# taaha-khan/2023-CompaCT-Image-Compression

Hardware: AMD Instinct MI355X
Metric: MPixels/s encode+decode, 12-bit 512x512 CT batch, bytes-exact (higher is better)
Workload: dtype u16

## Files before the change

### 2023-compact-image-compression_amd/csrc/deflate_kernels.hip

```cpp
#include <hip/hip_runtime.h>
#include <cstring>
#include <algorithm>

#include "cct_internal.h"
#include "wave_device.h"
#include "../../include/compact_hip.h"

namespace cct {
namespace {

constexpr int MIN_MATCH = 3, MAX_MATCH = 258, WSIZE = 32768;
constexpr int MIN_LOOKAHEAD = MAX_MATCH + MIN_MATCH + 1;
constexpr int MAX_DIST = WSIZE - MIN_LOOKAHEAD;
constexpr int TOO_FAR = 4096;
constexpr int BLOCK_SYMS = 16383;
constexpr int BLOCK_SYMS_ML9 = 32767;
constexpr int L_CODES = 286, D_CODES = 30, BL_CODES = 19, HEAP_SIZE = 2 * L_CODES + 1;
constexpr int END_BLOCK = 256, MAX_BITS = 15, MAX_BL_BITS = 7;
constexpr uint32_t Z_FILTERED = 1, Z_HUFFMAN_ONLY = 2, Z_RLE = 3, Z_FIXED = 4;
__host__ __device__ __forceinline__ bool short_pass(uint32_t strategy) { return strategy == Z_HUFFMAN_ONLY || strategy == Z_RLE; }

__constant__ uint8_t c_extra_lbits[29] = {0,0,0,0,0,0,0,0,1,1,1,1,2,2,2,2,3,3,3,3,4,4,4,4,5,5,5,5,0};
__constant__ uint8_t c_extra_dbits[30] = {0,0,0,0,1,1,2,2,3,3,4,4,5,5,6,6,7,7,8,8,9,9,10,10,11,11,12,12,13,13};
__constant__ uint8_t c_extra_blbits[19] = {0,0,0,0,0,0,0,0,0,0,0,0,0,0,0,0,2,3,7};
// ... 831 lines not shown
		const bool prev_eq = p >= 2 ? (rw >> 15) != 0 : (p == 1 && (rw0 & 0x7FFFu) >= 2u);
		const uint32_t run = rw & 0x7FFFu;
		uint32_t rec = 0, nxt = blk_end, cnt = 0;
		if (p < L) {
			const bool m = prev_eq && run >= (uint32_t)MIN_MATCH;
			rec = m ? (run << 8) | (1u << 17) : 0u;
			nxt = p + (m ? run : 1u);
			cnt = 1;
		}
		a.rec32[base + p] = rec;
#pragma unroll
		for (int r = 0; r < 6; r++) {
			const bool inside = nxt < blk_end;
			const int j = inside ? (int)(nxt - wb * 64) : lane;
			const uint32_t n2 = __shfl(nxt, j), c2 = __shfl(cnt, j);
			if (inside) { nxt = n2; cnt += c2; }
		}
		a.exit_pos[base + p] = (nxt - blk_end) | (cnt << 16);
	}
}

template <uint32_t BS>
__global__ void __launch_bounds__(256) dfl_huff_symbols_kernel(DeflateArgs a)
{
	const int s = blockIdx.y;
	const uint32_t L = a.in_sizes[s];
	const size_t base = (size_t)s * a.in_stride;
	const uint32_t *in4 = reinterpret_cast<const uint32_t *>(a.in + base);
	uint4 *sym4 = reinterpret_cast<uint4 *>(a.sym + base);
	uint32_t *bend = a.blk_end + (size_t)s * a.max_blocks, *btop = a.blk_top + (size_t)s * a.max_blocks;
	if (blockIdx.x == 0 && threadIdx.x == 0) a.total_syms[s] = L;
	const uint32_t nq = (L + 3) / 4;
	for (uint32_t q = blockIdx.x * blockDim.x + threadIdx.x; q < nq; q += gridDim.x * blockDim.x) {
		const uint32_t w = in4[q], p0 = 4 * q;
		uint32_t v[4];
#pragma unroll
		for (int k = 0; k < 4; k++) {
			const uint32_t p = p0 + (uint32_t)k;
			v[k] = p < L ? (w >> (8 * k)) & 255u : 0u;
			if (p < L && p % BS == BS - 1) { bend[p / BS] = p + 1; btop[p / BS] = p; }
		}
		sym4[q] = make_uint4(v[0], v[1], v[2], v[3]);
	}
}

#ifndef CCT_WALK_T
#define CCT_WALK_T 256
#endif
constexpr int WALK_T = CCT_WALK_T;
__global__ void __launch_bounds__(WALK_T) dfl_walk_kernel(DeflateArgs a, int n)
{
	__shared__ uint32_t s_land[WALK_T];
	__shared__ uint32_t s_wsum[WALK_T / 64];
	const int s = blockIdx.x;
	(void)n;
	const uint32_t L = a.in_sizes[s];
	const size_t base = (size_t)s * a.in_stride;
	const size_t bbase = (size_t)s * dfl_blk_words(a.in_stride);
	const uint32_t *exit_rec = a.exit_pos + base;
	const int tid = threadIdx.x;
	const uint32_t seg = (((L + WALK_T - 1) / WALK_T) + 63) & ~63u;
	const uint32_t seg_end = min(L, (uint32_t)(tid + 1) * seg);
	uint32_t start = min(L, (uint32_t)tid * seg), land = start, cnt = 0;
	auto hop_through = [&]() {
		uint32_t cur = start, c = 0;
		while (cur < seg_end) { const uint32_t e = exit_rec[cur]; c += e >> 16; cur = (cur & ~63u) + 64u + (e & 0xFFFFu); }
		land = cur; cnt = c;
	};
	hop_through();
	for (;;) {
		__syncthreads();
		s_land[tid] = land;
		__syncthreads();
		const uint32_t pl = tid ? s_land[tid - 1] : 0u;
		const bool moved = tid > 0 && pl != start;
		if (!__syncthreads_or(moved)) break;
		if (moved) { start = pl; hop_through(); }
	}
	uint32_t total;
	uint32_t syms = wg_excl_scan<WALK_T / 64>(cnt, s_wsum, total);
	if (tid == 0) a.total_syms[s] = total;
	for (uint32_t cur = start; cur < seg_end;) {
		const uint32_t b = cur >> 6;
		a.blk_entry[bbase + b] = cur;
		a.blk_symbase[bbase + b] = syms;
		const uint32_t e = exit_rec[cur];
		syms += e >> 16;
		cur = (cur & ~63u) + 64u + (e & 0xFFFFu);
	}
}

template <uint32_t BS>
__global__ void __launch_bounds__(256) dfl_symbols_kernel(DeflateArgs a)
{
	const int s = blockIdx.y;
	const uint32_t L = a.in_sizes[s];
	const uint8_t *in = a.in + (size_t)s * a.in_stride;
	const size_t base = (size_t)s * a.in_stride;
	const size_t bbase = (size_t)s * dfl_blk_words(a.in_stride);
	const uint32_t nblk64 = (L + 63) / 64;
	const int lane = threadIdx.x & 63;
	uint32_t *sym = a.sym + base;
	uint32_t *bend = a.blk_end + (size_t)s * a.max_blocks, *btop = a.blk_top + (size_t)s * a.max_blocks;
	const uint32_t lazy = short_pass(a.strategy) ? 0u : 1u;
	const uint32_t wb_step = gridDim.x * (blockDim.x >> 6), wb_last = nblk64 ? nblk64 - 1 : 0;
	struct Req { uint32_t entry, symbase, rec; uint8_t lit0; };
	auto request = [&](uint32_t wb) {
		const uint32_t wbc = min(wb, wb_last), pc = min(wbc * 64 + lane, L - 1);
		return Req{a.blk_entry[bbase + wbc], a.blk_symbase[bbase + wbc], a.rec32[base + pc], in[pc]};
	};
	const uint32_t wb0 = blockIdx.x * (blockDim.x >> 6) + (threadIdx.x >> 6);
	Req nx = nblk64 ? request(wb0) : Req{0xFFFFFFFFu, 0, 0, 0};
	for (uint32_t wb = wb0; wb < nblk64; wb += wb_step) {
		const uint32_t p = wb * 64 + lane;
		const Req cur_req = nx;
		nx = request(wb + wb_step);
		const uint32_t entry = cur_req.entry, symbase = cur_req.symbase;
		uint32_t rec = cur_req.rec;
		const uint8_t lit0 = cur_req.lit0;
		if (entry == 0xFFFFFFFFu) continue;
		if (p >= L) rec = 0;
		const uint32_t k = rec & 0xFFu, len = (rec >> 8) & 0x1FFu, dist = rec >> 17;
		const uint32_t nxt = len ? p + k + len : p + 1;
		const uint32_t cnt = len ? k + 1 : 1;
		const uint64_t jump = __ballot(len != 0);
		const uint32_t nvalid = min(64u, L - wb * 64);
		uint64_t visited = 0;
		uint32_t cur = (uint32_t)__builtin_amdgcn_readfirstlane((int)(entry - wb * 64));
		while (cur < nvalid) {
			const uint64_t rest = jump >> cur;
			if (!rest) { visited |= ~0ull << cur; break; }
			const int d = __ffsll((long long)rest) - 1;
			visited |= (d >= 63 ? ~0ull : ((2ull << d) - 1ull)) << cur;
			cur = (uint32_t)__builtin_amdgcn_readlane((int)nxt, (int)cur + d) - wb * 64;
		}
		if (nvalid < 64) visited &= (1ull << nvalid) - 1ull;
		const bool mine = (visited >> lane) & 1ull;
		const uint32_t v = mine ? cnt : 0u;
		uint32_t off = symbase + wave_incl_scan(v) - v;
		if (mine) {
			if (p == L - 1) a.postloop_lit[s] = 1;
			for (uint32_t t = 0; t < (len ? k : 1u); t++, off++) {
				sym[off] = t ? in[p + t] : lit0;
				if (off % BS == BS - 1) { bend[off / BS] = p + t + 1; btop[off / BS] = p + t + lazy; }
			}
			if (len) {
				sym[off] = (len - MIN_MATCH) | (dist << 16);
				if (off % BS == BS - 1) { bend[off / BS] = p + k + len; btop[off / BS] = p + k + lazy; }
			}
		}
	}
}

struct TreeScratch {
	uint16_t freq[HEAP_SIZE], dad[HEAP_SIZE], len[HEAP_SIZE], code[L_CODES + 2];
	uint16_t dfreq[2 * D_CODES + 1], ddad[2 * D_CODES + 1], dlen[2 * D_CODES + 1], dcode[D_CODES + 2];
	uint16_t bfreq[2 * BL_CODES + 1], bdad[2 * BL_CODES + 1], blen[2 * BL_CODES + 1], bcode[BL_CODES + 1];
	alignas(16) uint32_t heap[HEAP_SIZE + 11];
	uint32_t bl_count[MAX_BITS + 1];
	uint16_t next_code[MAX_BITS + 1];
	int heap_len, heap_max, max_code, overflow, lmax, dmax;
	uint32_t opt_len, static_len, dyn_body_bits;
	uint32_t hdr_bits[160];
	uint32_t hdr_nbits;
	int ntok, btype, max_blindex;
	uint8_t extra_l[29], extra_d[30], extra_bl[19], bl_order[19];
	__device__ __forceinline__ uint32_t *hist_l() { return heap; }
	__device__ __forceinline__ uint32_t *hist_d() { return heap + L_CODES + 2; }
	__device__ __forceinline__ uint8_t *length_code() { return reinterpret_cast<uint8_t *>(dad); }
	__device__ __forceinline__ uint8_t *dist_code() { return reinterpret_cast<uint8_t *>(dad) + 256; }
	__device__ __forceinline__ uint16_t *tok() { return dad; }
};
static_assert(sizeof(TreeScratch) <= 8192, "13 tree waves per CU: keep the working set around 8 KB");
static_assert(HEAP_SIZE >= L_CODES + D_CODES, "token list fits dad[]");
static_assert((HEAP_SIZE + 1) * 4 >= (L_CODES + 2 + D_CODES) * 4 && HEAP_SIZE * 2 >= 768, "aliases fit");
__device__ __forceinline__ uint32_t static_llen(int n) { return n <= 143 ? 8u : n <= 255 ? 9u : n <= 279 ? 7u : 8u; }

typedef __attribute__((address_space(3))) uint16_t lds_u16;
struct TreeView { lds_u16 *freq, *dad, *len, *code; };

__device__ __forceinline__ void pqdownheap(TreeScratch &S, int k, int hl)
{
	const uint32_t v = S.heap[k];
	for (int j = k << 1; j <= hl; j = k << 1) {
		const uint2 pr = *reinterpret_cast<const uint2 *>(&S.heap[j]);
		const int right = (j < hl && pr.y <= (pr.x | 1023u)) ? 1 : 0;
		const uint32_t e = right ? pr.y : pr.x;
		if (v <= (e | 1023u)) break;
		S.heap[k] = e;
		k = j + right;
	}
	S.heap[k] = v;
}

__device__ __forceinline__ TreeView view_of(TreeScratch &S, int kind)
{
	if (kind == 0) return TreeView{(lds_u16 *)S.freq, (lds_u16 *)S.dad, (lds_u16 *)S.len, (lds_u16 *)S.code};
	if (kind == 1) return TreeView{(lds_u16 *)S.dfreq, (lds_u16 *)S.ddad, (lds_u16 *)S.dlen, (lds_u16 *)S.dcode};
	return TreeView{(lds_u16 *)S.bfreq, (lds_u16 *)S.bdad, (lds_u16 *)S.blen, (lds_u16 *)S.bcode};
}
__device__ __forceinline__ int elems_of(int kind) { return kind == 0 ? L_CODES : kind == 1 ? D_CODES : BL_CODES; }

__device__ void tree_leaves(TreeScratch &S, int kind)
{
	const TreeView t = view_of(S, kind);
	const int lane = threadIdx.x, elems = elems_of(kind);
	const uint64_t lt_mask = (1ull << lane) - 1ull;
	int max_code = -1;
	uint32_t nleaf = 0;
	for (int n0 = 0; n0 < elems; n0 += 64) {
		const int n = n0 + lane;
		const uint32_t f = n < elems ? t.freq[n] : 0u;
		const uint64_t bal = __ballot(f != 0);
		if (f != 0) S.heap[1 + nleaf + (uint32_t)__popcll(bal & lt_mask)] = (f << 15) | (uint32_t)n;
		else if (n < elems) t.len[n] = 0;
		if (bal) max_code = n0 + 63 - __clzll((long long)bal);
		nleaf += (uint32_t)__popcll(bal);
	}
	if (lane == 0) { S.heap_len = (int)nleaf; S.max_code = max_code; }
}

constexpr int TREE_SIFTS = 8;
__device__ void tree_heap(TreeScratch &S, int kind)
{
	const TreeView t = view_of(S, kind);
	const int lane = threadIdx.x;
	int max_code = S.max_code, h = S.heap_len;
	while (h < 2) {
		const int node = max_code < 2 ? ++max_code : 0;
		h++;
		if (lane == 0) {
			t.freq[node] = 1; S.opt_len--;
			S.heap[h] = (1u << 15) | (uint32_t)node;
			if (kind == 0) S.static_len -= static_llen(node);
			else if (kind == 1) S.static_len -= 5;
		}
	}
	__syncthreads();
	for (int d = 31 - __clz(h >> 1); d >= 0; d--) {
		const int lo = 1 << d, hi = min((2 << d) - 1, h >> 1);
		for (int n0 = lo; n0 <= hi; n0 += 64) {
			if (n0 + lane <= hi) pqdownheap(S, n0 + lane, h);
			__builtin_amdgcn_wave_barrier();
		}
	}
	if (lane < TREE_SIFTS) {
		uint32_t v = 0, k = 1, hl = 0, w = 0;
		bool moving = false;
		const uint32_t sink = HEAP_SIZE + 3 + lane;
		auto tick = [&]() {
			const uint32_t j = k << 1;
			const uint2 pr = *reinterpret_cast<const uint2 *>(&S.heap[j]);
			const uint32_t right = (j < hl && pr.y <= (pr.x | 1023u)) ? 1u : 0u;
			const uint32_t e = right ? pr.y : pr.x;
			const bool go = moving && j <= hl && v > (e | 1023u);
			w = go ? e : v;
			uint32_t at = moving ? k : sink;
			asm volatile("" : "+v"(at), "+v"(w));
			S.heap[at] = w;
			k = go ? j + right : k;
			moving = go;
			__builtin_amdgcn_wave_barrier();
		};
		auto start = [&](int slot, uint32_t x) {
			const bool me = lane == slot;
			v = me ? x : v; k = me ? 1u : k; hl = me ? (uint32_t)h : hl; moving = moving || me;
		};
		int node = elems_of(kind), hm = HEAP_SIZE, slot = 0;
		uint32_t en = S.heap[1];
		for (;;) {
			while (__ballot(moving && ((uint32_t)h >> (__clz(k | 1u) - __clz(h))) == k)) tick();
			h--;
			start(slot, S.heap[h + 1]);
			tick();
			const uint32_t em = (uint32_t)__builtin_amdgcn_readlane((int)w, slot);
			const uint32_t f = (en >> 15) + (em >> 15);
			const uint32_t dn = (en >> 10) & 31u, dm = (em >> 10) & 31u;
			const uint32_t d = (dn >= dm ? dn : dm) + 1;
			if (lane == 0) {
				S.heap[hm - 1] = en; S.heap[hm - 2] = em;
				t.freq[node] = (uint16_t)f;
				t.dad[en & 1023u] = t.dad[em & 1023u] = (uint16_t)node;
			}
			hm -= 2;
			slot = (slot + 1) & (TREE_SIFTS - 1);
			tick();
			start(slot, (f << 15) | (d << 10) | (uint32_t)node);
			tick();
			en = (uint32_t)__builtin_amdgcn_readlane((int)w, slot);
			slot = (slot + 1) & (TREE_SIFTS - 1);
			node++;
			if (h < 2) break;
			tick();
		}
		while (__ballot(moving)) tick();
		if (lane == 0) {
			S.heap[--hm] = en;
			S.heap_len = h; S.heap_max = hm;
			S.max_code = max_code;
		}
	}
}

__device__ void tree_depths(TreeScratch &S, int kind)
{
	const TreeView t = view_of(S, kind);
	const int lane = threadIdx.x;
	const int max_length = kind == 2 ? MAX_BL_BITS : MAX_BITS;
	const int base = kind == 0 ? 257 : 0;
	const int max_code = S.max_code, heap_max = S.heap_max;
	const uint32_t root = S.heap[heap_max];
	constexpr uint16_t UNKNOWN = 0xFFFF;
	for (int h = heap_max + 1 + lane; h < HEAP_SIZE; h += 64) t.len[S.heap[h] & 1023u] = UNKNOWN;
	if (lane == 0) t.len[root & 1023u] = 0;
	if (lane <= MAX_BITS) S.bl_count[lane] = 0;
	__syncthreads();
	for (bool again = true; again;) {
		again = false;
		for (int h0 = heap_max + 1; h0 < HEAP_SIZE; h0 += 64) {
			const int h = h0 + lane;
			bool unknown = false;
			if (h < HEAP_SIZE) {
				const int n = (int)(S.heap[h] & 1023u);
				if (t.len[n] == UNKNOWN) {
					const uint32_t ld = t.len[t.dad[n]];
					if (ld == UNKNOWN) unknown = true;
					else t.len[n] = (uint16_t)min(ld + 1u, (uint32_t)max_length);
				}
			}
			if (__ballot(unknown)) again = true;
		}
		__syncthreads();
	}
	int overflow = 0;
	for (int h0 = heap_max + 1; h0 < HEAP_SIZE; h0 += 64) {
		const int h = h0 + lane;
		const bool clamped = h < HEAP_SIZE && t.len[t.dad[S.heap[h] & 1023u]] == (uint32_t)max_length;
		overflow += (int)__popcll(__ballot(clamped));
	}
	uint32_t o = 0, st = 0;
	for (int n = lane; n <= max_code; n += 64) {
		const uint32_t f = t.freq[n];
		if (f == 0) continue;
		const uint32_t bits = t.len[n];
		atomicAdd(&S.bl_count[bits], 1u);
		uint32_t xbits = 0;
		if (n >= base) xbits = kind == 0 ? S.extra_l[n - base] : kind == 1 ? S.extra_d[n] : S.extra_bl[n];
		o += f * (bits + xbits);
		if (kind == 0) st += f * (static_llen(n) + xbits);
		else if (kind == 1) st += f * (5u + xbits);
	}
	o = wave_sum(o); st = wave_sum(st);
	if (lane == 0) { S.overflow = overflow; S.opt_len += o; S.static_len += st; }
}

__device__ void tree_fix(TreeScratch &S, int kind)
{
	const TreeView t = view_of(S, kind);
	const int max_length = kind == 2 ? MAX_BL_BITS : MAX_BITS;
	const int max_code = S.max_code;
	int overflow = S.overflow;
	if (overflow > 0) {
		int bits, n, m, h = HEAP_SIZE;
		do {
			bits = max_length - 1;
			while (S.bl_count[bits] == 0) bits--;
			S.bl_count[bits]--; S.bl_count[bits + 1] += 2; S.bl_count[max_length]--;
			overflow -= 2;
		} while (overflow > 0);
		for (bits = max_length; bits != 0; bits--) {
			n = (int)S.bl_count[bits];
			while (n != 0) {
				m = (int)(S.heap[--h] & 1023u);
				if (m > max_code) continue;
				if ((uint32_t)t.len[m] != (uint32_t)bits) {
					S.opt_len += ((uint32_t)bits - t.len[m]) * t.freq[m];
					t.len[m] = (uint16_t)bits;
				}
				n--;
			}
		}
	}
	uint32_t code = 0;
	for (int bits = 1; bits <= MAX_BITS; bits++) { code = (code + S.bl_count[bits - 1]) << 1; S.next_code[bits] = (uint16_t)code; }
}

__device__ void tree_codes(TreeScratch &S, int kind)
{
	const TreeView t = view_of(S, kind);
	const int lane = threadIdx.x, max_code = S.max_code;
	const uint64_t lt_mask = (1ull << lane) - 1ull;
	uint32_t seen[MAX_BITS + 1];
#pragma unroll
	for (int b = 1; b <= MAX_BITS; b++) seen[b] = S.next_code[b];
	for (int n0 = 0; n0 <= max_code; n0 += 64) {
		const int n = n0 + lane;
		const int len = n <= max_code ? (int)t.len[n] : 0;
		uint32_t mine = 0;
#pragma unroll
		for (int b = 1; b <= MAX_BITS; b++) {
			const uint64_t bal = __ballot(len == b);
			if (len == b) mine = seen[b] + (uint32_t)__popcll(bal & lt_mask);
			seen[b] += (uint32_t)__popcll(bal);
		}
		if (len != 0) t.code[n] = (uint16_t)(__brev(mine) >> (32 - len));
	}
}

__device__ void scan_tree_wave(TreeScratch &S, const TreeView &t, int max_code)
{
	const int lane = threadIdx.x;
	constexpr int NCH = (L_CODES + 63) / 64;
	const int n_el = max_code + 1;
	uint32_t v[NCH];
	uint64_t startmask[NCH];
#pragma unroll
	for (int c = 0; c < NCH; c++) {
		const int n = c * 64 + lane;
		v[c] = n < n_el ? (uint32_t)t.len[n] : 0xFFFFu;
		const uint32_t before = n == 0 ? 0xFFFFFFFFu : (uint32_t)t.len[max(n - 1, 0)];
		startmask[c] = __ballot(n < n_el && v[c] != before);
	}
	uint16_t *tk = S.tok();
	uint32_t base = (uint32_t)S.ntok;
#pragma unroll
	for (int c = 0; c < NCH; c++) {
		if (c * 64 >= n_el) break;
		const int n = c * 64 + lane;
		const bool start = (startmask[c] >> lane) & 1ull;
		uint32_t R = 0;
		if (start) {
			int nxt = n_el;
			const uint64_t rest = lane < 63 ? startmask[c] >> (lane + 1) : 0ull;
			if (rest) nxt = n + (int)__ffsll((long long)rest);
			else {
#pragma unroll
				for (int c2 = NCH - 1; c2 > c; c2--) if (startmask[c2]) nxt = min(nxt, c2 * 64 + (int)__ffsll((long long)startmask[c2]) - 1);
			}
			R = (uint32_t)(nxt - n);
		}
		const uint32_t val = v[c];
		uint32_t nlit_head = 0, nrep6 = 0, tail_lit = 0, tail_sym = 0xFFFFFFFFu, nbig = 0;
		if (start) {
			if (val != 0) {
				if (R < 4) nlit_head = R;
				else if (R <= 6) { nlit_head = 1; tail_sym = 16u | ((R - 4u) << 5); }
				else {
					nlit_head = 1; nrep6 = 1 + (R - 7u) / 6u;
					const uint32_t r = (R - 7u) % 6u;
					if (r < 3) tail_lit = r; else tail_sym = 16u | ((r - 3u) << 5);
				}
			} else {
				nbig = R / 138u;
				const uint32_t r = R % 138u;
				if (r < 3) tail_lit = r;
				else if (r <= 10) tail_sym = 17u | ((r - 3u) << 5);
				else tail_sym = 18u | ((r - 11u) << 5);
			}
		}
		const uint32_t ntok = nlit_head + nrep6 + nbig + tail_lit + (tail_sym != 0xFFFFFFFFu ? 1u : 0u);
		uint32_t chunk_tok;
		const uint32_t ex = wave_excl_scan(ntok, chunk_tok);
		if (start) {
			uint32_t w = base + ex;
			for (uint32_t i = 0; i < nlit_head; i++) tk[w++] = (uint16_t)val;
			for (uint32_t i = 0; i < nrep6; i++) tk[w++] = (uint16_t)(16u | (3u << 5));
			for (uint32_t i = 0; i < nbig; i++) tk[w++] = (uint16_t)(18u | (127u << 5));
			for (uint32_t i = 0; i < tail_lit; i++) tk[w++] = (uint16_t)val;
			if (tail_sym != 0xFFFFFFFFu) tk[w++] = (uint16_t)tail_sym;
			if (nlit_head + tail_lit) atomicAdd(&S.hdr_bits[val], nlit_head + tail_lit);
			if (nrep6) atomicAdd(&S.hdr_bits[16], nrep6);
			if (nbig) atomicAdd(&S.hdr_bits[18], nbig);
			if (tail_sym != 0xFFFFFFFFu) atomicAdd(&S.hdr_bits[tail_sym & 31u], 1u);
		}
		base += chunk_tok;
	}
	if (lane == 0) S.ntok = (int)base;
}

__device__ __forceinline__ void hdr_or(TreeScratch &S, uint32_t pos, uint32_t value, uint32_t n)
{
	const uint32_t w = pos >> 5, sh = pos & 31u;
	atomicOr(&S.hdr_bits[w], value << sh);
	if (sh + n > 32u) atomicOr(&S.hdr_bits[w + 1], value >> (32u - sh));
}

__device__ void send_header(TreeScratch &S)
{
	const int lane = threadIdx.x;
	const int nbl = S.max_blindex + 1;
	if (lane == 0) hdr_or(S, 0, (uint32_t)(S.lmax + 1 - 257) | ((uint32_t)(S.dmax + 1 - 1) << 5) | ((uint32_t)(nbl - 4) << 10), 14);
	if (lane < nbl) hdr_or(S, 14u + 3u * (uint32_t)lane, S.blen[S.bl_order[lane]], 3);
	uint32_t base = 14u + 3u * (uint32_t)nbl;
	const uint16_t *tk = S.tok();
	const int nt = S.ntok;
	for (int c0 = 0; c0 < nt; c0 += 64) {
		const int i = c0 + lane;
		uint32_t nbits = 0, val = 0;
		if (i < nt) {
			const uint32_t sym = tk[i] & 31u, ex = tk[i] >> 5;
			const uint32_t cl = S.blen[sym];
			nbits = cl + S.extra_bl[sym];
			val = (uint32_t)S.bcode[sym] | (ex << cl);
		}
		uint32_t chunk_bits;
		const uint32_t ex = wave_excl_scan(nbits, chunk_bits);
		if (nbits) hdr_or(S, base + ex, val, nbits);
		base += chunk_bits;
	}
	if (lane == 0) S.hdr_nbits = base;
}

constexpr int TREE_BLOCKS = 1;

__device__ __forceinline__ uint32_t window_base(uint32_t top, uint32_t L, uint32_t strategy)
{
	const uint32_t lam = strategy == Z_HUFFMAN_ONLY ? 0u : strategy == Z_RLE ? (uint32_t)MAX_MATCH : (uint32_t)MIN_LOOKAHEAD - 1u;
	const uint32_t kf = L >= 65536u ? (L - 65536u) / 32768u + 1u : 0u;
	uint32_t k = 0;
	if (top >= 65536u - lam) k = min((top - (65536u - lam)) / 32768u + 1u, kf);
	if (k == kf && 32768u * k + (uint32_t)(WSIZE + MAX_DIST) <= top && L <= top + lam) k++;
	return 32768u * k;
}
__global__ void __launch_bounds__(64) dfl_tree_kernel(DeflateArgs a)
{
	__shared__ TreeScratch S4[TREE_BLOCKS];
	const int s = blockIdx.y, m0 = blockIdx.x * TREE_BLOCKS, lane = threadIdx.x;
	const uint32_t T = a.total_syms[s];
	const uint32_t L = a.in_sizes[s];
	const uint32_t BS = a.block_syms;
	uint32_t nfull = T / BS;
	if (T % BS == 0 && nfull > 0 && !short_pass(a.strategy) && a.postloop_lit[s]) nfull--;
	const uint32_t nblocks = nfull + 1;
	BlockMeta *meta = a.block_meta + (size_t)s * a.max_blocks;
	if ((uint32_t)m0 >= nblocks) return;
	const int nb = (int)min((uint32_t)TREE_BLOCKS, nblocks - (uint32_t)m0);
	const uint32_t *bend = a.blk_end + (size_t)s * a.max_blocks;
	const bool owner = lane < nb;
#ifdef CCT_TREE_PROF
	long long tp[16]; int tpi = 0;
#define TREE_STAMP() do { if (tpi < 16) tp[tpi++] = clock64(); } while (0)
#else
#define TREE_STAMP() do {} while (0)
#endif
	TREE_STAMP();

	for (int q = 0; q < nb; q++) {
		TreeScratch &S = S4[q];
		const int m = m0 + q;
		const bool last = (uint32_t)m == nblocks - 1;
		const uint32_t first = (uint32_t)m * BS;
		const uint32_t nsym = last ? T - first : BS;
		const uint32_t *sym = a.sym + (size_t)s * a.in_stride + first;
		for (int i = lane; i < HEAP_SIZE; i += 64) { S.freq[i] = 0; S.len[i] = 0; }
		for (int i = lane; i < L_CODES + 2; i += 64) S.code[i] = 0;
		for (int i = lane; i < 2 * D_CODES + 1; i += 64) { S.dfreq[i] = 0; S.dlen[i] = 0; S.ddad[i] = 0; }
		for (int i = lane; i < D_CODES + 2; i += 64) S.dcode[i] = 0;
		for (int i = lane; i < 2 * BL_CODES + 1; i += 64) { S.bfreq[i] = 0; S.blen[i] = 0; S.bdad[i] = 0; }
		for (int i = lane; i < BL_CODES + 1; i += 64) S.bcode[i] = 0;
		uint8_t *length_code = S.length_code(), *dist_code = S.dist_code();
		{
			uint8_t dc[8], lc4[4];
#pragma unroll
			for (int k = 0; k < 8; k++) dc[k] = c_dist_code[lane + 64 * k];
#pragma unroll
			for (int k = 0; k < 4; k++) lc4[k] = c_length_code[lane + 64 * k];
			const int l29 = min(lane, 28), l30 = min(lane, 29), l19 = min(lane, 18);
			const uint8_t xl = c_extra_lbits[l29], xd = c_extra_dbits[l30], xb = c_extra_blbits[l19], bo = c_bl_order[l19];
#pragma unroll
			for (int k = 0; k < 8; k++) dist_code[lane + 64 * k] = dc[k];
#pragma unroll
			for (int k = 0; k < 4; k++) length_code[lane + 64 * k] = lc4[k];
			if (lane < 29) S.extra_l[lane] = xl;
			if (lane < 30) S.extra_d[lane] = xd;
			if (lane < 19) { S.extra_bl[lane] = xb; S.bl_order[lane] = bo; }
		}
		uint32_t *hl = S.hist_l(), *hd = S.hist_d();
		for (int i = lane; i < L_CODES; i += 64) hl[i] = 0;
		if (lane < D_CODES) hd[lane] = 0;
		__syncthreads();
		{
			const uint32_t lasts = nsym ? nsym - 1 : 0;
			uint32_t nv[16];
#pragma unroll
			for (int k = 0; k < 16; k++) nv[k] = sym[min((uint32_t)(k * 64 + lane), lasts)];
			for (uint32_t i0 = 0; i0 < nsym; i0 += 64 * 16) {
				uint32_t v[16];
#pragma unroll
				for (int k = 0; k < 16; k++) v[k] = nv[k];
#pragma unroll
				for (int k = 0; k < 16; k++) nv[k] = sym[min(i0 + 1024u + (uint32_t)(k * 64 + lane), lasts)];
#pragma unroll
				for (int k = 0; k < 16; k++) {
					if (i0 + (uint32_t)(k * 64 + lane) >= nsym) continue;
					const uint32_t dist = v[k] >> 16, lc = v[k] & 0xFFu;
					if (dist == 0) atomicAdd(&hl[lc], 1u);
					else {
						const uint32_t d1 = dist - 1;
						atomicAdd(&hl[length_code[lc] + 256 + 1], 1u);
						atomicAdd(&hd[d1 < 256 ? dist_code[d1] : dist_code[256 + (d1 >> 7)]], 1u);
					}
				}
			}
		}
		__syncthreads();
		for (int i = lane; i < L_CODES; i += 64) S.freq[i] = (uint16_t)hl[i];
		if (lane < D_CODES) S.dfreq[lane] = (uint16_t)hd[lane];
		for (int i = lane; i < 160; i += 64) S.hdr_bits[i] = 0;
		if (lane == 0) { S.opt_len = 0; S.static_len = 0; S.hdr_nbits = 0; S.ntok = 0; S.btype = 0; S.max_blindex = 0; }
		__syncthreads();
		if (lane == 0) S.freq[END_BLOCK] = 1;
		for (int i = lane; i < HEAP_SIZE; i += 64) S.dad[i] = 0;
	}
	__syncthreads();
	TREE_STAMP();
#pragma unroll 1
	for (int kind = 0; kind < 3; kind++) {
		if (kind == 2) {
			if (owner) S4[lane].dyn_body_bits = S4[lane].opt_len;
			__syncthreads();
			for (int q = 0; q < nb; q++) {
				TreeScratch &S = S4[q];
				scan_tree_wave(S, view_of(S, 0), S.lmax);
				__syncthreads();
				scan_tree_wave(S, view_of(S, 1), S.dmax);
				__syncthreads();
				if (lane < BL_CODES) { S.bfreq[lane] = (uint16_t)S.hdr_bits[lane]; S.hdr_bits[lane] = 0; }
			}
			__syncthreads();
		}
		for (int q = 0; q < nb; q++) tree_leaves(S4[q], kind);
		__syncthreads();
		TREE_STAMP();
		for (int q = 0; q < nb; q++) tree_heap(S4[q], kind);
		__syncthreads();
		TREE_STAMP();
		for (int q = 0; q < nb; q++) tree_depths(S4[q], kind);
		__syncthreads();
		if (owner) {
			tree_fix(S4[lane], kind);
			if (kind == 0) S4[lane].lmax = S4[lane].max_code; else if (kind == 1) S4[lane].dmax = S4[lane].max_code;
		}
		__syncthreads();
		for (int q = 0; q < nb; q++) tree_codes(S4[q], kind);
		__syncthreads();
		TREE_STAMP();
	}
	if (owner) {
		TreeScratch &S = S4[lane];
		const int m = m0 + lane;
		const bool last = (uint32_t)m == nblocks - 1;
		const uint32_t first = (uint32_t)m * BS;
		const uint32_t nsym = last ? T - first : BS;
		const uint32_t in_begin = m == 0 ? 0u : bend[m - 1];
		const uint32_t in_end = last ? L : bend[m];
		int max_blindex;
		for (max_blindex = BL_CODES - 1; max_blindex >= 3; max_blindex--)
			if (S.blen[S.bl_order[max_blindex]] != 0) break;
		S.opt_len += 3 * ((uint32_t)max_blindex + 1) + 5 + 5 + 4;
		uint32_t opt_lenb = (S.opt_len + 3 + 7) >> 3;
		const uint32_t static_lenb = (S.static_len + 3 + 7) >> 3;
		if (static_lenb <= opt_lenb) opt_lenb = static_lenb;
		const uint32_t stored_len = in_end - in_begin;
		const bool in_window = in_begin >= window_base(last ? L : a.blk_top[(size_t)s * a.max_blocks + m], L, a.strategy);
		BlockMeta bm;
		bm.in_begin = in_begin; bm.stored_len = stored_len; bm.first_sym = first; bm.nsym = nsym; bm.last = last ? 1u : 0u;
		if (in_window && stored_len + 4 <= opt_lenb) {
			bm.type = 0; bm.hdr_nbits = 0; bm.body_bits = 0;
		} else if (a.strategy == Z_FIXED || static_lenb == opt_lenb) {
			bm.type = 1; bm.hdr_nbits = 0; bm.body_bits = S.static_len;
		} else {
			bm.type = 2; bm.hdr_nbits = 0;
			bm.body_bits = S.dyn_body_bits;
		}
		S.btype = (int)bm.type; S.max_blindex = max_blindex;
		meta[m] = bm;
		if (m == 0) a.n_blocks[s] = nblocks;
	}
	__syncthreads();
	for (int q = 0; q < nb; q++) {
		TreeScratch &S = S4[q];
		if (S.btype != 2) continue;
		send_header(S);
		__syncthreads();
		BlockTables *bt = a.block_tables + ((size_t)s * a.max_blocks + m0 + q);
		for (int i = lane; i * 32 < (int)S.hdr_nbits; i += 64) bt->hdr_bits[i] = S.hdr_bits[i];
		if (lane == 0) meta[m0 + q].hdr_nbits = S.hdr_nbits;
	}
	__syncthreads();
	TREE_STAMP();
#ifdef CCT_TREE_PROF
	if (s == 0 && m0 == 0 && lane == 0) {
		printf("[tree prof] nb=%d:", nb);
		for (int i = 1; i < tpi; i++) printf(" %lld", tp[i] - tp[i - 1]);
		printf("  (hist | leaves0 heap0 rest0 | scan+leaves1 heap1 rest1 | scan_tree+leaves2 heap2 rest2 | final)\n");
	}
#endif
	for (int q = 0; q < nb; q++) {
		TreeScratch &S = S4[q];
		BlockTables *bt = a.block_tables + ((size_t)s * a.max_blocks + m0 + q);
		for (int i = lane; i < L_CODES; i += 64) { bt->lcode[i] = S.code[i]; bt->llen[i] = (uint8_t)S.len[i]; }
		if (lane < D_CODES) { bt->dcode[lane] = S.dcode[lane]; bt->dlen[lane] = (uint8_t)S.dlen[lane]; }
	}
}

__global__ void __launch_bounds__(256) dfl_adler_kernel(DeflateArgs a)
{
	__shared__ unsigned long long sa[256], sb[256];
	const int s = blockIdx.x;
	const uint32_t L = a.in_sizes[s];
	const uint8_t *in = a.in + (size_t)s * a.in_stride;
	unsigned long long A = 0, B = 0;
	const uint32_t nfull = L / 16;
	constexpr int U = 8;
	for (uint32_t g0 = threadIdx.x; g0 < nfull; g0 += blockDim.x * U) {
		uint4 v[U];
#pragma unroll
		for (int u = 0; u < U; u++) v[u] = *reinterpret_cast<const uint4 *>(in + (size_t)min(g0 + (uint32_t)u * blockDim.x, nfull - 1) * 16);
#pragma unroll
		for (int u = 0; u < U; u++) {
			const uint32_t g = g0 + (uint32_t)u * blockDim.x;
			if (g >= nfull) continue;
			const uint32_t w[4] = {v[u].x, v[u].y, v[u].z, v[u].w};
			uint32_t sd = 0, sk = 0;
#pragma unroll
			for (int k = 0; k < 16; k++) { const uint32_t d = (w[k >> 2] >> ((k & 3) * 8)) & 0xFFu; sd += d; sk += (uint32_t)k * d; }
			A += sd;
			B += (unsigned long long)(L - g * 16) * sd - sk;
		}
	}
	if (threadIdx.x == 0)
		for (uint32_t i = nfull * 16; i < L; i++) { const unsigned long long d = in[i]; A += d; B += (unsigned long long)(L - i) * d; }
	sa[threadIdx.x] = A; sb[threadIdx.x] = B;
	__syncthreads();
	for (int st = 128; st > 0; st >>= 1) {
		if ((int)threadIdx.x < st) { sa[threadIdx.x] += sa[threadIdx.x + st]; sb[threadIdx.x] += sb[threadIdx.x + st]; }
		__syncthreads();
	}
	if (threadIdx.x == 0) {
		const uint32_t lo = (uint32_t)((1ull + sa[0]) % 65521ull);
		const uint32_t hi = (uint32_t)(((unsigned long long)L + sb[0]) % 65521ull);
		a.adler[s] = (hi << 16) | lo;
	}
}

__global__ void __launch_bounds__(64) dfl_layout_kernel(DeflateArgs a, int n)
{
	const int s = blockIdx.x, lane = threadIdx.x;
	if (s >= n) return;
	uint8_t *out = a.out + (size_t)s * a.out_stride;
	BlockMeta *meta = a.block_meta + (size_t)s * a.max_blocks;
	const uint32_t nb = a.n_blocks[s];
	const uint32_t ad = a.adler[s];
	uint64_t bit = 8ull * 15;
	for (uint32_t m0 = 0; m0 < nb; m0 += 64) {
		const uint32_t m = m0 + (uint32_t)lane, cnt = min(64u, nb - m0);
		const BlockMeta bm = meta[min(m, nb - 1)];
		const uint32_t flags = (bm.type == 0 ? 1u : 0u) | (bm.last ? 2u : 0u);
		const uint64_t size = bm.type == 0 ? 32 + 8ull * bm.stored_len : 3ull + bm.hdr_nbits + bm.body_bits;
		uint64_t mine = 0;
		for (uint32_t j = 0; j < cnt; j++) {
			const uint32_t fj = __shfl(flags, (int)j);
			const uint64_t zj = __shfl((unsigned long long)size, (int)j);
			if (j == (uint32_t)lane) mine = bit;
			bit = (fj & 1u) ? ((bit + 3 + 7) & ~7ull) + zj : bit + zj;
			if (fj & 2u) bit = (bit + 7) & ~7ull;
		}
		if (m < nb) meta[m].bit_off = mine;
	}
	if (lane == 0) {
		for (int i = 0; i < 13; i++) out[i] = a.header13[i];
		out[13] = 0x78; out[14] = (uint8_t)a.zlib_flg;
		const uint64_t byte = bit >> 3;
		out[byte + 0] = (uint8_t)(ad >> 24); out[byte + 1] = (uint8_t)(ad >> 16);
		out[byte + 2] = (uint8_t)(ad >> 8);  out[byte + 3] = (uint8_t)ad;
		a.out_sizes[s] = (uint32_t)(byte + 4);
	}
}

__device__ __forceinline__ void or_bits(uint32_t *words, uint64_t bit, uint64_t value, int nbits)
{
	if (nbits == 0) return;
	const uint64_t w = bit >> 5;
	const int sh = (int)(bit & 31);
	const uint64_t lo = value << sh;
	const uint64_t hi = sh ? (value >> (64 - sh)) : 0ull;
	atomicOr(&words[w], (uint32_t)lo);
	if (sh + nbits > 32) atomicOr(&words[w + 1], (uint32_t)(lo >> 32));
	if (sh + nbits > 64) atomicOr(&words[w + 2], (uint32_t)hi);
}

#ifndef CCT_EMIT_K
#define CCT_EMIT_K 4
#endif
constexpr int EMIT_K = CCT_EMIT_K;
constexpr int EMIT_T = 256 * EMIT_K;
constexpr int EMIT_LIMBS = (EMIT_K * 48 + 63) / 64;
constexpr int EMIT_WBUF = EMIT_T * 48 / 32 + 8;
__global__ void __launch_bounds__(256) dfl_emit_kernel(DeflateArgs a)
{
	__shared__ uint32_t wsum[2][4];
	const int s = blockIdx.y, m = blockIdx.x;
	if ((uint32_t)m >= a.n_blocks[s]) return;
	const BlockMeta bm = a.block_meta[(size_t)s * a.max_blocks + m];
	const BlockTables *bt = a.block_tables + ((size_t)s * a.max_blocks + m);
	uint8_t *out = a.out + (size_t)s * a.out_stride;
	uint32_t *words = reinterpret_cast<uint32_t *>(out);
	const uint8_t *in = a.in + (size_t)s * a.in_stride;
	uint64_t bit = bm.bit_off;
	if (bm.type == 0) {
		if (threadIdx.x == 0) or_bits(words, bit, (uint64_t)bm.last, 3);
		const uint64_t byte = ((bit + 3 + 7) & ~7ull) >> 3;
		if (threadIdx.x == 0) {
			out[byte] = (uint8_t)(bm.stored_len & 0xFF); out[byte + 1] = (uint8_t)(bm.stored_len >> 8);
			out[byte + 2] = (uint8_t)(~bm.stored_len & 0xFF); out[byte + 3] = (uint8_t)((~bm.stored_len >> 8) & 0xFF);
		}
		for (uint32_t i = threadIdx.x; i < bm.stored_len; i += blockDim.x) out[byte + 4 + i] = in[bm.in_begin + i];
		return;
	}
	if (threadIdx.x == 0) or_bits(words, bit, (uint64_t)((bm.type << 1) + bm.last), 3);
	bit += 3;
	if (bm.type == 2) {
		for (uint32_t i = threadIdx.x; i * 32 < bm.hdr_nbits; i += blockDim.x) {
			const int nb = (int)min(32u, bm.hdr_nbits - i * 32);
			or_bits(words, bit + 32ull * i, bt->hdr_bits[i], nb);
		}
		bit += bm.hdr_nbits;
	}
	const uint32_t *sym = a.sym + (size_t)s * a.in_stride + bm.first_sym;
	const bool dyn = bm.type == 2;
	const int lane = threadIdx.x & 63, wave = threadIdx.x >> 6;
	__shared__ uint16_t t_lcode[L_CODES + 2], t_dcode[D_CODES + 2];
	__shared__ uint8_t t_llen[L_CODES + 2], t_dlen[D_CODES + 2];
	__shared__ uint32_t wbuf[2][EMIT_WBUF];
	__shared__ uint8_t t_length_code[256], t_dist_code[512], t_extra_l[32], t_extra_d[32];
	__shared__ uint16_t t_base_length[32], t_base_dist[32];
	{
		const int t = threadIdx.x, t2 = min(t + 256, L_CODES - 1), td = min(t, D_CODES - 1), t29 = min(t, 28), t30 = min(t, 29);
		const uint16_t *lsrc = dyn ? bt->lcode : c_static_lcode, *dsrc = dyn ? bt->dcode : c_static_dcode;
		const uint8_t *llsrc = dyn ? bt->llen : c_static_llen;
		const uint16_t lc0 = lsrc[t], lc1 = lsrc[t2];
		const uint8_t ll0 = llsrc[t], ll1 = llsrc[t2];
		const uint16_t dc = dsrc[td];
		uint8_t dl = bt->dlen[td];
		if (!dyn) dl = 5;
		const uint8_t k0 = c_dist_code[t], k1 = c_dist_code[t + 256], lcd = c_length_code[t];
		const uint8_t xl = c_extra_lbits[t29], xd = c_extra_dbits[t30];
		const uint16_t bl = c_base_length[t29], bd = c_base_dist[t30];
// ... 366 lines not shown
```

Measured before the change: 17500.

## Build literal and distance Huffman heaps concurrently and parallelize depth computation

Gives the distance tree its own heap region and per-kind heap_len/max_code/heap_max slots, so the literal and distance heaps are built together in one pass using 16 sift lanes (8 per tree). Tree depth assignment switches from repeated full rescans to a register-cached chunked level propagation, and the cost sums are computed from values preloaded into registers. The histogram loop now precomputes length and distance codes and skips the bounds check on full chunks. Together these cut the serial, latency-bound tree-building phase per deflate block, at the cost of more LDS per TreeScratch, more registers, and more intricate lane bookkeeping.

```diff
diff --git a/2023-compact-image-compression_amd/csrc/deflate_kernels.hip b/2023-compact-image-compression_amd/csrc/deflate_kernels.hip
--- a/2023-compact-image-compression_amd/csrc/deflate_kernels.hip
+++ b/2023-compact-image-compression_amd/csrc/deflate_kernels.hip
@@ -1007,16 +1007,20 @@
 	}
 }
 
+constexpr int DHEAP = HEAP_SIZE + 11, DHEAP_SIZE = 2 * D_CODES + 1;
+constexpr int HDR_WORDS = 144;
+static_assert(DHEAP % 2 == 0, "child pairs are read as one 64-bit word");
 struct TreeScratch {
 	uint16_t freq[HEAP_SIZE], dad[HEAP_SIZE], len[HEAP_SIZE], code[L_CODES + 2];
 	uint16_t dfreq[2 * D_CODES + 1], ddad[2 * D_CODES + 1], dlen[2 * D_CODES + 1], dcode[D_CODES + 2];
 	uint16_t bfreq[2 * BL_CODES + 1], bdad[2 * BL_CODES + 1], blen[2 * BL_CODES + 1], bcode[BL_CODES + 1];
-	alignas(16) uint32_t heap[HEAP_SIZE + 11];
+	alignas(16) uint32_t heap[HEAP_SIZE + 11 + DHEAP_SIZE + 11];
 	uint32_t bl_count[MAX_BITS + 1];
 	uint16_t next_code[MAX_BITS + 1];
-	int heap_len, heap_max, max_code, overflow, lmax, dmax;
+	int heap_len[2], heap_max[2], max_code[2];
+	int overflow, lmax, dmax;
 	uint32_t opt_len, static_len, dyn_body_bits;
-	uint32_t hdr_bits[160];
+	uint32_t hdr_bits[HDR_WORDS];
 	uint32_t hdr_nbits;
 	int ntok, btype, max_blindex;
 	uint8_t extra_l[29], extra_d[30], extra_bl[19], bl_order[19];
@@ -1032,20 +1036,21 @@
 __device__ __forceinline__ uint32_t static_llen(int n) { return n <= 143 ? 8u : n <= 255 ? 9u : n <= 279 ? 7u : 8u; }
 
 typedef __attribute__((address_space(3))) uint16_t lds_u16;
+typedef __attribute__((address_space(3))) uint8_t lds_u8;
 struct TreeView { lds_u16 *freq, *dad, *len, *code; };
 
-__device__ __forceinline__ void pqdownheap(TreeScratch &S, int k, int hl)
-{
-	const uint32_t v = S.heap[k];
+__device__ __forceinline__ void pqdownheap(uint32_t *heap, int k, int hl)
+{
+	const uint32_t v = heap[k];
 	for (int j = k << 1; j <= hl; j = k << 1) {
-		const uint2 pr = *reinterpret_cast<const uint2 *>(&S.heap[j]);
+		const uint2 pr = *reinterpret_cast<const uint2 *>(&heap[j]);
 		const int right = (j < hl && pr.y <= (pr.x | 1023u)) ? 1 : 0;
 		const uint32_t e = right ? pr.y : pr.x;
 		if (v <= (e | 1023u)) break;
-		S.heap[k] = e;
+		heap[k] = e;
 		k = j + right;
 	}
-	S.heap[k] = v;
+	heap[k] = v;
 }
 
 __device__ __forceinline__ TreeView view_of(TreeScratch &S, int kind)
@@ -1055,11 +1060,15 @@
 	return TreeView{(lds_u16 *)S.bfreq, (lds_u16 *)S.bdad, (lds_u16 *)S.blen, (lds_u16 *)S.bcode};
 }
 __device__ __forceinline__ int elems_of(int kind) { return kind == 0 ? L_CODES : kind == 1 ? D_CODES : BL_CODES; }
+__device__ __forceinline__ int heap_base(int kind) { return kind == 1 ? DHEAP : 0; }
+__device__ __forceinline__ int heap_end(int kind) { return kind == 1 ? DHEAP_SIZE : HEAP_SIZE; }
+__device__ __forceinline__ int slot_of(int kind) { return kind == 1 ? 1 : 0; }
 
 __device__ void tree_leaves(TreeScratch &S, int kind)
 {
 	const TreeView t = view_of(S, kind);
 	const int lane = threadIdx.x, elems = elems_of(kind);
+	uint32_t *heap = S.heap + heap_base(kind);
 	const uint64_t lt_mask = (1ull << lane) - 1ull;
 	int max_code = -1;
 	uint32_t nleaf = 0;
@@ -1067,50 +1076,68 @@
 		const int n = n0 + lane;
 		const uint32_t f = n < elems ? t.freq[n] : 0u;
 		const uint64_t bal = __ballot(f != 0);
-		if (f != 0) S.heap[1 + nleaf + (uint32_t)__popcll(bal & lt_mask)] = (f << 15) | (uint32_t)n;
+		if (f != 0) heap[1 + nleaf + (uint32_t)__popcll(bal & lt_mask)] = (f << 15) | (uint32_t)n;
 		else if (n < elems) t.len[n] = 0;
 		if (bal) max_code = n0 + 63 - __clzll((long long)bal);
 		nleaf += (uint32_t)__popcll(bal);
 	}
-	if (lane == 0) { S.heap_len = (int)nleaf; S.max_code = max_code; }
+	if (lane == 0) { S.heap_len[slot_of(kind)] = (int)nleaf; S.max_code[slot_of(kind)] = max_code; }
 }
 
 constexpr int TREE_SIFTS = 8;
-__device__ void tree_heap(TreeScratch &S, int kind)
+__device__ void tree_heapify(TreeScratch &S, int kind)
 {
 	const TreeView t = view_of(S, kind);
-	const int lane = threadIdx.x;
-	int max_code = S.max_code, h = S.heap_len;
+	const int lane = threadIdx.x, sl = slot_of(kind);
+	uint32_t *heap = S.heap + heap_base(kind);
+	int max_code = __builtin_amdgcn_readfirstlane(S.max_code[sl]), h = __builtin_amdgcn_readfirstlane(S.heap_len[sl]);
+	const bool forced = h < 2;
 	while (h < 2) {
 		const int node = max_code < 2 ? ++max_code : 0;
 		h++;
 		if (lane == 0) {
 			t.freq[node] = 1; S.opt_len--;
-			S.heap[h] = (1u << 15) | (uint32_t)node;
+			heap[h] = (1u << 15) | (uint32_t)node;
 			if (kind == 0) S.static_len -= static_llen(node);
 			else if (kind == 1) S.static_len -= 5;
 		}
 	}
+	if (forced && lane == 0) { S.heap_len[sl] = h; S.max_code[sl] = max_code; }
 	__syncthreads();
 	for (int d = 31 - __clz(h >> 1); d >= 0; d--) {
 		const int lo = 1 << d, hi = min((2 << d) - 1, h >> 1);
 		for (int n0 = lo; n0 <= hi; n0 += 64) {
-			if (n0 + lane <= hi) pqdownheap(S, n0 + lane, h);
+			if (n0 + lane <= hi) pqdownheap(heap, n0 + lane, h);
 			__builtin_amdgcn_wave_barrier();
 		}
 	}
-	if (lane < TREE_SIFTS) {
+}
+
+template <int NH>
+__device__ void tree_heap(TreeScratch &S, int kind0)
+{
+	const int lane = threadIdx.x;
+#pragma unroll
+	for (int q = 0; q < NH; q++) tree_heapify(S, kind0 + q);
+	__syncthreads();
+	if (lane < TREE_SIFTS * NH) {
+		const int grp = NH == 2 ? lane >> 3 : 0, kind = kind0 + grp, sl = slot_of(kind), sub = lane & (TREE_SIFTS - 1);
+		const TreeView t = view_of(S, kind);
+		const uint32_t hb = (uint32_t)heap_base(kind);
+		int h = S.heap_len[sl], hm = heap_end(kind), node = elems_of(kind);
+		uint32_t en = S.heap[hb + 1];
+		bool active = true;
 		uint32_t v = 0, k = 1, hl = 0, w = 0;
 		bool moving = false;
-		const uint32_t sink = HEAP_SIZE + 3 + lane;
+		const uint32_t sink = hb + (uint32_t)heap_end(kind) + 3 + (uint32_t)sub;
 		auto tick = [&]() {
 			const uint32_t j = k << 1;
-			const uint2 pr = *reinterpret_cast<const uint2 *>(&S.heap[j]);
+			const uint2 pr = *reinterpret_cast<const uint2 *>(&S.heap[hb + j]);
 			const uint32_t right = (j < hl && pr.y <= (pr.x | 1023u)) ? 1u : 0u;
 			const uint32_t e = right ? pr.y : pr.x;
 			const bool go = moving && j <= hl && v > (e | 1023u);
 			w = go ? e : v;
-			uint32_t at = moving ? k : sink;
+			uint32_t at = moving ? hb + k : sink;
 			asm volatile("" : "+v"(at), "+v"(w));
 			S.heap[at] = w;
 			k = go ? j + right : k;
@@ -1118,43 +1145,85 @@
 			__builtin_amdgcn_wave_barrier();
 		};
 		auto start = [&](int slot, uint32_t x) {
-			const bool me = lane == slot;
+			const bool me = active && sub == slot;
 			v = me ? x : v; k = me ? 1u : k; hl = me ? (uint32_t)h : hl; moving = moving || me;
 		};
-		int node = elems_of(kind), hm = HEAP_SIZE, slot = 0;
-		uint32_t en = S.heap[1];
+		auto root_of = [&](int slot) {
+			const uint32_t r0 = (uint32_t)__builtin_amdgcn_readlane((int)w, slot);
+			if (NH == 1) return r0;
+			const uint32_t r1 = (uint32_t)__builtin_amdgcn_readlane((int)w, slot + TREE_SIFTS);
+			return grp ? r1 : r0;
+		};
+		int slot = 0;
 		for (;;) {
-			while (__ballot(moving && ((uint32_t)h >> (__clz(k | 1u) - __clz(h))) == k)) tick();
-			h--;
-			start(slot, S.heap[h + 1]);
+			while (__ballot(active && moving && ((uint32_t)h >> (__clz(k | 1u) - __clz(h))) == k)) tick();
+			const uint32_t last = S.heap[hb + (uint32_t)h];
+			h -= active ? 1 : 0;
+			start(slot, last);
 			tick();
-			const uint32_t em = (uint32_t)__builtin_amdgcn_readlane((int)w, slot);
+			const uint32_t em = root_of(slot);
 			const uint32_t f = (en >> 15) + (em >> 15);
 			const uint32_t dn = (en >> 10) & 31u, dm = (em >> 10) & 31u;
 			const uint32_t d = (dn >= dm ? dn : dm) + 1;
-			if (lane == 0) {
-				S.heap[hm - 1] = en; S.heap[hm - 2] = em;
+			if (sub == 0 && active) {
+				S.heap[hb + hm - 1] = en; S.heap[hb + hm - 2] = em;
 				t.freq[node] = (uint16_t)f;
 				t.dad[en & 1023u] = t.dad[em & 1023u] = (uint16_t)node;
 			}
-			hm -= 2;
+			hm -= active ? 2 : 0;
 			slot = (slot + 1) & (TREE_SIFTS - 1);
 			tick();
 			start(slot, (f << 15) | (d << 10) | (uint32_t)node);
 			tick();
-			en = (uint32_t)__builtin_amdgcn_readlane((int)w, slot);
+			const uint32_t r = root_of(slot);
+			en = active ? r : en;
 			slot = (slot + 1) & (TREE_SIFTS - 1);
-			node++;
-			if (h < 2) break;
+			node += active ? 1 : 0;
+			active = active && h >= 2;
+			if (!__ballot(active)) break;
 			tick();
 		}
 		while (__ballot(moving)) tick();
-		if (lane == 0) {
-			S.heap[--hm] = en;
-			S.heap_len = h; S.heap_max = hm;
-			S.max_code = max_code;
-		}
-	}
+		if (sub == 0) {
+			S.heap[hb + --hm] = en;
+			S.heap_len[sl] = h; S.heap_max[sl] = hm;
+		}
+	}
+}
+
+template <int NCH>
+__device__ __forceinline__ int tree_levels(const uint32_t *heap, int heap_end, const TreeView &t, int heap_max, int max_length)
+{
+	static_assert(9 * 64 >= HEAP_SIZE - 1, "nine chunks hold every tail");
+	constexpr uint16_t UNKNOWN = 0xFFFF;
+	const int lane = threadIdx.x;
+	const uint32_t root = heap[heap_max];
+	uint32_t nd[NCH];
+	uint32_t pending = 0;
+#pragma unroll
+	for (int c = 0; c < NCH; c++) nd[c] = heap[min(heap_max + 1 + c * 64 + lane, heap_end - 1)] & 1023u;
+#pragma unroll
+	for (int c = 0; c < NCH; c++) nd[c] |= (uint32_t)t.dad[nd[c]] << 16;
+#pragma unroll
+	for (int c = 0; c < NCH; c++)
+		if (heap_max + 1 + c * 64 + lane < heap_end) { t.len[nd[c] & 0xFFFFu] = UNKNOWN; pending |= 1u << c; }
+	if (lane == 0) t.len[root & 1023u] = 0;
+	__syncthreads();
+	int overflow = 0;
+	while (__ballot(pending != 0)) {
+		uint32_t ld[NCH];
+#pragma unroll
+		for (int c = 0; c < NCH; c++) ld[c] = (uint32_t)t.len[nd[c] >> 16];
+#pragma unroll
+		for (int c = 0; c < NCH; c++) {
+			if (!((pending >> c) & 1u) || ld[c] == UNKNOWN) continue;
+			t.len[nd[c] & 0xFFFFu] = (uint16_t)min(ld[c] + 1u, (uint32_t)max_length);
+			overflow += ld[c] == (uint32_t)max_length ? 1 : 0;
+			pending &= ~(1u << c);
+		}
+		__syncthreads();
+	}
+	return overflow;
 }
 
 __device__ void tree_depths(TreeScratch &S, int kind)
@@ -1163,45 +1232,36 @@
 	const int lane = threadIdx.x;
 	const int max_length = kind == 2 ? MAX_BL_BITS : MAX_BITS;
 	const int base = kind == 0 ? 257 : 0;
-	const int max_code = S.max_code, heap_max = S.heap_max;
-	const uint32_t root = S.heap[heap_max];
-	constexpr uint16_t UNKNOWN = 0xFFFF;
-	for (int h = heap_max + 1 + lane; h < HEAP_SIZE; h += 64) t.len[S.heap[h] & 1023u] = UNKNOWN;
-	if (lane == 0) t.len[root & 1023u] = 0;
+	const int max_code = __builtin_amdgcn_readfirstlane(S.max_code[slot_of(kind)]);
+	const int heap_max = __builtin_amdgcn_readfirstlane(S.heap_max[slot_of(kind)]);
+	const uint32_t *heap = S.heap + heap_base(kind);
+	const int he = heap_end(kind);
+	const int nch = (he - 1 - heap_max + 63) >> 6;
 	if (lane <= MAX_BITS) S.bl_count[lane] = 0;
-	__syncthreads();
-	for (bool again = true; again;) {
-		again = false;
-		for (int h0 = heap_max + 1; h0 < HEAP_SIZE; h0 += 64) {
-			const int h = h0 + lane;
-			bool unknown = false;
-			if (h < HEAP_SIZE) {
-				const int n = (int)(S.heap[h] & 1023u);
-				if (t.len[n] == UNKNOWN) {
-					const uint32_t ld = t.len[t.dad[n]];
-					if (ld == UNKNOWN) unknown = true;
-					else t.len[n] = (uint16_t)min(ld + 1u, (uint32_t)max_length);
-				}
-			}
-			if (__ballot(unknown)) again = true;
-		}
-		__syncthreads();
-	}
-	int overflow = 0;
-	for (int h0 = heap_max + 1; h0 < HEAP_SIZE; h0 += 64) {
-		const int h = h0 + lane;
-		const bool clamped = h < HEAP_SIZE && t.len[t.dad[S.heap[h] & 1023u]] == (uint32_t)max_length;
-		overflow += (int)__popcll(__ballot(clamped));
+	int overflow = nch <= 1 ? tree_levels<1>(heap, he, t, heap_max, max_length)
+	             : nch <= 4 ? tree_levels<4>(heap, he, t, heap_max, max_length) : tree_levels<9>(heap, he, t, heap_max, max_length);
+	overflow = (int)wave_sum((uint32_t)overflow);
+	constexpr int LCH = (L_CODES + 63) / 64;
+	const int lch = (max_code + 64) >> 6;
+	const lds_u8 *xtab = kind == 0 ? (lds_u8 *)S.extra_l : kind == 1 ? (lds_u8 *)S.extra_d : (lds_u8 *)S.extra_bl;
+	const int xlast = kind == 0 ? L_CODES - 257 - 1 : kind == 1 ? D_CODES - 1 : BL_CODES - 1;
+	uint32_t fr[LCH], bl[LCH], xb[LCH];
+#pragma unroll
+	for (int c = 0; c < LCH; c++) {
+		const int n = min(c * 64 + lane, max_code);
+		fr[c] = c < lch ? (uint32_t)t.freq[n] : 0u;
+		bl[c] = c < lch ? (uint32_t)t.len[n] : 0u;
+		xb[c] = c < lch ? (uint32_t)xtab[min(max(n - base, 0), xlast)] : 0u;
 	}
 	uint32_t o = 0, st = 0;
-	for (int n = lane; n <= max_code; n += 64) {
-		const uint32_t f = t.freq[n];
+#pragma unroll
+	for (int c = 0; c < LCH; c++) {
+		const int n = c * 64 + lane;
+		const uint32_t f = n <= max_code ? fr[c] : 0u;
 		if (f == 0) continue;
-		const uint32_t bits = t.len[n];
-		atomicAdd(&S.bl_count[bits], 1u);
-		uint32_t xbits = 0;
-		if (n >= base) xbits = kind == 0 ? S.extra_l[n - base] : kind == 1 ? S.extra_d[n] : S.extra_bl[n];
-		o += f * (bits + xbits);
+		atomicAdd(&S.bl_count[bl[c]], 1u);
+		const uint32_t xbits = n >= base ? xb[c] : 0u;
+		o += f * (bl[c] + xbits);
 		if (kind == 0) st += f * (static_llen(n) + xbits);
 		else if (kind == 1) st += f * (5u + xbits);
 	}
@@ -1213,10 +1273,11 @@
 {
 	const TreeView t = view_of(S, kind);
 	const int max_length = kind == 2 ? MAX_BL_BITS : MAX_BITS;
-	const int max_code = S.max_code;
+	const int max_code = S.max_code[slot_of(kind)];
+	const uint32_t *heap = S.heap + heap_base(kind);
 	int overflow = S.overflow;
 	if (overflow > 0) {
-		int bits, n, m, h = HEAP_SIZE;
+		int bits, n, m, h = heap_end(kind);
 		do {
 			bits = max_length - 1;
 			while (S.bl_count[bits] == 0) bits--;
@@ -1226,7 +1287,7 @@
 		for (bits = max_length; bits != 0; bits--) {
 			n = (int)S.bl_count[bits];
 			while (n != 0) {
-				m = (int)(S.heap[--h] & 1023u);
+				m = (int)(heap[--h] & 1023u);
 				if (m > max_code) continue;
 				if ((uint32_t)t.len[m] != (uint32_t)bits) {
 					S.opt_len += ((uint32_t)bits - t.len[m]) * t.freq[m];
@@ -1243,7 +1304,7 @@
 __device__ void tree_codes(TreeScratch &S, int kind)
 {
 	const TreeView t = view_of(S, kind);
-	const int lane = threadIdx.x, max_code = S.max_code;
+	const int lane = threadIdx.x, max_code = S.max_code[slot_of(kind)];
 	const uint64_t lt_mask = (1ull << lane) - 1ull;
 	uint32_t seen[MAX_BITS + 1];
 #pragma unroll
@@ -1445,23 +1506,30 @@
 				for (int k = 0; k < 16; k++) v[k] = nv[k];
 #pragma unroll
 				for (int k = 0; k < 16; k++) nv[k] = sym[min(i0 + 1024u + (uint32_t)(k * 64 + lane), lasts)];
+				uint32_t code[16];
 #pragma unroll
 				for (int k = 0; k < 16; k++) {
-					if (i0 + (uint32_t)(k * 64 + lane) >= nsym) continue;
-					const uint32_t dist = v[k] >> 16, lc = v[k] & 0xFFu;
-					if (dist == 0) atomicAdd(&hl[lc], 1u);
-					else {
-						const uint32_t d1 = dist - 1;
-						atomicAdd(&hl[length_code[lc] + 256 + 1], 1u);
-						atomicAdd(&hd[d1 < 256 ? dist_code[d1] : dist_code[256 + (d1 >> 7)]], 1u);
-					}
+					const uint32_t d1 = (v[k] >> 16) - 1u;
+					code[k] = (uint32_t)length_code[v[k] & 0xFFu] | (uint32_t)dist_code[d1 < 256 ? d1 : 256 + ((d1 >> 7) & 255u)] << 16;
+				}
+				auto count = [&](int k) {
+					const bool match = (v[k] >> 16) != 0;
+					atomicAdd(&hl[match ? (code[k] & 0xFFFFu) + 256 + 1 : v[k] & 0xFFu], 1u);
+					if (match) atomicAdd(&hd[code[k] >> 16], 1u);
+				};
+				if (i0 + 1024u <= nsym) {
+#pragma unroll
+					for (int k = 0; k < 16; k++) count(k);
+				} else {
+#pragma unroll
+					for (int k = 0; k < 16; k++) if (i0 + (uint32_t)(k * 64 + lane) < nsym) count(k);
 				}
 			}
 		}
 		__syncthreads();
 		for (int i = lane; i < L_CODES; i += 64) S.freq[i] = (uint16_t)hl[i];
 		if (lane < D_CODES) S.dfreq[lane] = (uint16_t)hd[lane];
-		for (int i = lane; i < 160; i += 64) S.hdr_bits[i] = 0;
+		for (int i = lane; i < HDR_WORDS; i += 64) S.hdr_bits[i] = 0;
 		if (lane == 0) { S.opt_len = 0; S.static_len = 0; S.hdr_nbits = 0; S.ntok = 0; S.btype = 0; S.max_blindex = 0; }
 		__syncthreads();
 		if (lane == 0) S.freq[END_BLOCK] = 1;
@@ -1484,17 +1552,18 @@
 			}
 			__syncthreads();
 		}
-		for (int q = 0; q < nb; q++) tree_leaves(S4[q], kind);
+		if (kind != 1) for (int q = 0; q < nb; q++) { tree_leaves(S4[q], kind); if (kind == 0) tree_leaves(S4[q], 1); }
 		__syncthreads();
 		TREE_STAMP();
-		for (int q = 0; q < nb; q++) tree_heap(S4[q], kind);
+		if (kind == 0) for (int q = 0; q < nb; q++) tree_heap<2>(S4[q], 0);
+		if (kind == 2) for (int q = 0; q < nb; q++) tree_heap<1>(S4[q], 2);
 		__syncthreads();
 		TREE_STAMP();
 		for (int q = 0; q < nb; q++) tree_depths(S4[q], kind);
 		__syncthreads();
 		if (owner) {
 			tree_fix(S4[lane], kind);
-			if (kind == 0) S4[lane].lmax = S4[lane].max_code; else if (kind == 1) S4[lane].dmax = S4[lane].max_code;
+			if (kind == 0) S4[lane].lmax = S4[lane].max_code[0]; else if (kind == 1) S4[lane].dmax = S4[lane].max_code[1];
 		}
 		__syncthreads();
 		for (int q = 0; q < nb; q++) tree_codes(S4[q], kind);
@@ -1548,7 +1617,7 @@
 	if (s == 0 && m0 == 0 && lane == 0) {
 		printf("[tree prof] nb=%d:", nb);
 		for (int i = 1; i < tpi; i++) printf(" %lld", tp[i] - tp[i - 1]);
-		printf("  (hist | leaves0 heap0 rest0 | scan+leaves1 heap1 rest1 | scan_tree+leaves2 heap2 rest2 | final)\n");
+		printf("  (hist | leaves0+1 heap0+1 rest0 | - - rest1 | scan_tree+leaves2 heap2 rest2 | final)\n");
 	}
 #endif
 	for (int q = 0; q < nb; q++) {
```

After: 17750 (median of 6 runs). 1.01x the previous value.
